# dusk-network/plonk

Hardware: NVIDIA H100
Metric: proofs/sec @ 2^16 gates (higher is better)
Workload: dtype u32 limbs (Fr 256-bit / Fp 384-bit Montgomery)

## Files before the change

### plonk_b200/csrc/msm.cu

```cuda
#include <algorithm>
#include <atomic>
#include <vector>

#include "common.cuh"
#include "fp_inv.cuh"
#include "g1.cuh"
#include "host_field.h"

struct pb200_srs {
  size_t n_points;
  int c;
  int W;
  uint4* table;
};

namespace pb {

static constexpr int kGroup = 8;
static constexpr unsigned kHeavyMin = 32, kHeavyFactor = 4;
static constexpr unsigned kHeavyChunk = 256, kHeavyChunkWide = 1024;

PB_D G1Affine ld_affine(const uint4* p, size_t i) {
  const uint4* q = p + 6 * i;
  uint4 a0 = __ldg(q), a1 = __ldg(q + 1), a2 = __ldg(q + 2), b0 = __ldg(q + 3), b1 = __ldg(q + 4), b2 = __ldg(q + 5);
  G1Affine r;
  r.x.v[0] = a0.x; r.x.v[1] = a0.y; r.x.v[2] = a0.z; r.x.v[3] = a0.w;
  r.x.v[4] = a1.x; r.x.v[5] = a1.y; r.x.v[6] = a1.z; r.x.v[7] = a1.w;
  r.x.v[8] = a2.x; r.x.v[9] = a2.y; r.x.v[10] = a2.z; r.x.v[11] = a2.w;
  r.y.v[0] = b0.x; r.y.v[1] = b0.y; r.y.v[2] = b0.z; r.y.v[3] = b0.w;
  r.y.v[4] = b1.x; r.y.v[5] = b1.y; r.y.v[6] = b1.z; r.y.v[7] = b1.w;
  r.y.v[8] = b2.x; r.y.v[9] = b2.y; r.y.v[10] = b2.z; r.y.v[11] = b2.w;
  return r;
}
PB_D void st_fp(uint4* q, const Fp& f) {
  q[0] = make_uint4(f.v[0], f.v[1], f.v[2], f.v[3]);
  q[1] = make_uint4(f.v[4], f.v[5], f.v[6], f.v[7]);
  q[2] = make_uint4(f.v[8], f.v[9], f.v[10], f.v[11]);
}
PB_D Fp ld_fp(const uint4* q) {
  uint4 a = q[0], b = q[1], c = q[2];
  Fp f;
  f.v[0] = a.x; f.v[1] = a.y; f.v[2] = a.z; f.v[3] = a.w;
  f.v[4] = b.x; f.v[5] = b.y; f.v[6] = b.z; f.v[7] = b.w;
  f.v[8] = c.x; f.v[9] = c.y; f.v[10] = c.z; f.v[11] = c.w;
  return f;
}
PB_D void st_affine(uint4* p, size_t i, const G1Affine& a) {
  st_fp(p + 6 * i, a.x);
  st_fp(p + 6 * i + 3, a.y);
}
PB_D void st_xyzz(uint4* p, size_t i, const G1Xyzz& a) {
  st_fp(p + 12 * i, a.x);
// ... 162 lines not shown
  s = s.from_mont();
  const unsigned mask = (1u << c) - 1u, half = 1u << (c - 1);
  unsigned carry = 0;
  for (int w = 0; w < W; w++) {
    const int bit = w * c;
    const int word = bit >> 5, off = bit & 31;
    unsigned val = 0;
    if (word < 8) {
      val = s.v[word] >> off;
      if (off && word + 1 < 8) val |= s.v[word + 1] << (32 - off);
      val &= mask;
    }
    unsigned d = val + carry;
    unsigned sign = 0;
    if (d > half) {
      d = (1u << c) - d;
      sign = 1;
      carry = 1;
    } else {
      carry = 0;
    }
    const size_t slot = ((size_t)b * W + w) * n + i;
    if (d == 0) {
      ebkt[slot] = 0xffffffffu;
    } else {
      const unsigned bucket = d - 1;
      ebkt[slot] = (bucket << 1) | sign;
      epos[slot] = atomicAdd(&counts[(size_t)b * nb + bucket], 1u);
    }
  }
}

__global__ void __launch_bounds__(1024) k_msm_scan(const unsigned* counts, unsigned* offsets, unsigned* order, unsigned* n_heavy,
                                                   unsigned* heavy_pre, unsigned* max_len, unsigned nb, int size_shift,
                                                   unsigned heavy_chunk) {
  __shared__ unsigned sums[1024];
  __shared__ unsigned bins[1024];
  __shared__ unsigned s_nh, s_total, s_thr_units, s_max;
  const unsigned b = blockIdx.x, tid = threadIdx.x;
  const unsigned* cnt = counts + (size_t)b * nb;
  unsigned* off = offsets + (size_t)b * (nb + 1);
  unsigned* ord = order + (size_t)b * nb;
  const unsigned chunk = (nb + 1023) / 1024;
  const unsigned lo = tid * chunk, hi = min(nb, lo + chunk);
  unsigned s = 0, mx = 0;
  for (unsigned k = lo; k < hi; k++) {
    s += cnt[k];
    mx = max(mx, cnt[k]);
  }
  sums[tid] = s;
  bins[tid] = 0;
  if (tid == 0) s_max = 0;
  __syncthreads();
  if (mx) atomicMax(&s_max, mx);
  for (unsigned d = 1; d < 1024; d <<= 1) {
    unsigned v = (tid >= d) ? sums[tid - d] : 0;
    __syncthreads();
    sums[tid] += v;
    __syncthreads();
  }
  unsigned run = sums[tid] - s;
  for (unsigned k = lo; k < hi; k++) {
    off[k] = run;
    run += cnt[k];
  }
  if (tid == 1023) {
    off[nb] = sums[1023];
    s_total = sums[1023];
    max_len[b] = s_max;
  }
  for (unsigned k = tid; k < nb; k += 1024) atomicAdd(&bins[1023u - min(cnt[k] >> size_shift, 1023u)], 1u);
  __syncthreads();
  const unsigned mine = bins[tid];
  sums[tid] = mine;
  __syncthreads();
  for (unsigned d = 1; d < 1024; d <<= 1) {
    unsigned v = (tid >= d) ? sums[tid - d] : 0;
    __syncthreads();
    sums[tid] += v;
    __syncthreads();
  }
  bins[tid] = sums[tid] - mine;
  if (tid == 0) {
    const unsigned avg = s_total / nb;
    const unsigned thr = max(kHeavyMin, kHeavyFactor * avg);
    s_thr_units = min(1021u, (thr + (1u << size_shift) - 1u) >> size_shift);
  }
  __syncthreads();
  if (tid == 1022u - s_thr_units) {
    n_heavy[b] = sums[tid];
    s_nh = sums[tid];
  }
  __syncthreads();
  for (unsigned k = tid; k < nb; k += 1024) {
    const unsigned pos = atomicAdd(&bins[1023u - min(cnt[k] >> size_shift, 1023u)], 1u);
    ord[pos] = k;
  }
  __syncthreads();
  const unsigned nh = s_nh;
  unsigned* hp = heavy_pre + (size_t)b * (nb + 1);
  const unsigned per = (nh + 1023u) / 1024u;
  const unsigned h_lo = min(nh, tid * per), h_hi = min(nh, h_lo + per);
  unsigned c = 0;
  for (unsigned h = h_lo; h < h_hi; h++) c += (cnt[ord[h]] + heavy_chunk - 1) / heavy_chunk;
  sums[tid] = c;
  __syncthreads();
  for (unsigned d = 1; d < 1024; d <<= 1) {
    unsigned v = (tid >= d) ? sums[tid - d] : 0;
    __syncthreads();
    sums[tid] += v;
    __syncthreads();
  }
  unsigned run2 = sums[tid] - c;
  for (unsigned h = h_lo; h < h_hi; h++) {
    hp[h] = run2;
    run2 += (cnt[ord[h]] + heavy_chunk - 1) / heavy_chunk;
  }
  if (tid == 1023) hp[nh] = sums[1023];
}

__global__ void k_msm_scatter(const unsigned* ebkt, const unsigned* epos, const unsigned* offsets, size_t n,
                              int W, unsigned nb, size_t n_table, size_t first, unsigned* sorted) {
  size_t i = (size_t)blockIdx.x * blockDim.x + threadIdx.x;
  if (i >= n) return;
  const unsigned w = blockIdx.y, b = blockIdx.z;
  const size_t slot = ((size_t)b * W + w) * n + i;
  const unsigned e = ebkt[slot];
  if (e == 0xffffffffu) return;
  const unsigned bucket = e >> 1, sign = e & 1u;
  const unsigned dst = offsets[(size_t)b * (nb + 1) + bucket] + epos[slot];
  sorted[(size_t)b * n * W + dst] = (unsigned)(((size_t)w * n_table + first + i) << 1) | sign;
}

PB_D G1Xyzz shfl_down_xyzz(const G1Xyzz& p, int delta, int width) {
  G1Xyzz r;
#pragma unroll
  for (int i = 0; i < 12; i++) {
    r.x.v[i] = __shfl_down_sync(0xffffffffu, p.x.v[i], delta, width);
    r.y.v[i] = __shfl_down_sync(0xffffffffu, p.y.v[i], delta, width);
    r.zz.v[i] = __shfl_down_sync(0xffffffffu, p.zz.v[i], delta, width);
    r.zzz.v[i] = __shfl_down_sync(0xffffffffu, p.zzz.v[i], delta, width);
  }
  return r;
}

template <int THREADS, int MIN_CTAS>
__global__ void __launch_bounds__(THREADS, MIN_CTAS) k_msm_accumulate(const uint4* table, const unsigned* sorted,
                                                               const unsigned* offsets, const unsigned* order,
                                                               const unsigned* n_heavy, unsigned nb, int log_split, size_t cap,
                                                               uint4* sums) {
  const size_t t = (size_t)blockIdx.x * blockDim.x + threadIdx.x;
  const unsigned split = 1u << log_split;
  const unsigned b = blockIdx.y;
  const bool valid = t < ((size_t)nb << log_split) && (t >> log_split) >= n_heavy[b];
  const unsigned part = (unsigned)t & (split - 1);
  unsigned bucket = 0, lo = 0, hi = 0;
  if (valid) {
    bucket = order[(size_t)b * nb + (t >> log_split)];
    const unsigned* off = offsets + (size_t)b * (nb + 1);
    const unsigned start = off[bucket], end = off[bucket + 1];
    const unsigned chunk = (end - start + split - 1) >> log_split;
    lo = min(end, start + part * chunk);
    hi = min(end, lo + chunk);
  }
  const unsigned* src = sorted + (size_t)b * cap;
  G1Xyzz acc = G1Xyzz::identity();
  unsigned e_next = 0;
  G1Affine p_next;
  if (lo < hi) {
    e_next = __ldg(src + lo);
    p_next = ld_affine(table, e_next >> 1);
  }
  for (unsigned k = lo; k < hi; k++) {
    const unsigned e = e_next;
    G1Affine p = p_next;
    if (k + 1 < hi) {
      e_next = __ldg(src + k + 1);
      p_next = ld_affine(table, e_next >> 1);
    }
    if (p.is_inf()) continue;
    if (e & 1u) p.y = p.y.neg();
    xyzz_madd(acc, p.x, p.y);
  }
  for (int d = (int)split >> 1; d > 0; d >>= 1) {
    G1Xyzz o = shfl_down_xyzz(acc, d, (int)split);
    xyzz_add(acc, o);
  }
  if (valid && part == 0) st_xyzz(sums, (size_t)b * nb + bucket, acc);
}

PB_D G1Xyzz warp_sum(G1Xyzz v) {
// ... 591 lines not shown
  *g_out = g;
  return 0;
}
static int msm_plan(const pb200_srs* srs, uint32_t batch, MsmTail* tail, unsigned* n_groups_out, int* g_out) {
  return msm_plan_c(srs->c, batch, tail, n_groups_out, g_out);
}

static unsigned reduction_chunks(const DigitPlan& plan, unsigned n_groups, unsigned n_parts) {
  unsigned chunks = (n_parts + kListChunk - 1) / kListChunk;
  for (int j = 0; j < plan.ndig; j++) chunks = std::max(chunks, ((n_groups >> plan.bits[j]) + kListChunk - 1) / kListChunk);
  return std::max(chunks, 1u);
}

static int msm_enqueue(const pb200_srs* srs, size_t first, const uint64_t* d_scalars, size_t n, uint32_t batch, size_t stride,
                       cudaStream_t st, ScratchScope& scope, uint4** d_result, MsmTail* tail, cudaEvent_t* prof_ev,
                       const unsigned** d_totals) {
  if (first + n > srs->n_points) return fail(PB200_ERR_DEGREE_TOO_LARGE, "more scalars than commit-key points");
  const int c = srs->c, W = srs->W;
  const unsigned nb = 1u << (c - 1);
  const size_t cap = n * (size_t)W;
  if (((srs->n_points * (size_t)W) << 1) >= ((size_t)1 << 32)) return fail(PB200_ERR_INVALID_ARG, "commit key too large for 32-bit point references");
  unsigned n_groups = 0;
  int g = 0;
  PB_TRY(msm_plan(srs, batch, tail, &n_groups, &g));
  const DigitPlan& plan = tail->plan;
  uint4* result = nullptr;
  PB_ALLOC(scope, result, (size_t)batch * (plan.ndig + 1) * 192);
  *d_result = result;
  if (n == 0) {
    PB_CUDA(cudaMemsetAsync(result, 0, (size_t)batch * (plan.ndig + 1) * 192, st));
    return 0;
  }

  int log_split = 0;
  if (!t_msm_throughput_hint) {
    const size_t avg = cap / nb;
    while (log_split < 5 && ((size_t)nb * batch << log_split) < (1u << 17) && (avg >> (log_split + 1)) >= 8) log_split++;
  }
  if (const char* env = getenv("PB200_MSM_LOG_SPLIT")) log_split = atoi(env);

  unsigned *counts = nullptr, *offsets = nullptr, *order = nullptr, *ebkt = nullptr, *epos = nullptr, *sorted = nullptr;
  uint4 *sums = nullptr, *lists = nullptr, *S = nullptr, *P = nullptr;
  PB_ALLOC(scope, counts, (size_t)batch * nb * 4);
  PB_ALLOC(scope, offsets, (size_t)batch * (nb + 1) * 4);
  PB_ALLOC(scope, order, (size_t)batch * nb * 4);
  const bool affine = msm_affine_enabled();
  unsigned *n_heavy = nullptr, *heavy_pre = nullptr, *max_len = nullptr;
  PB_ALLOC(scope, max_len, (size_t)batch * 4);
  PB_ALLOC(scope, n_heavy, (size_t)batch * 4);
  PB_ALLOC(scope, heavy_pre, (size_t)batch * (nb + 1) * 4);
  PB_ALLOC(scope, ebkt, (size_t)batch * cap * 4);
  PB_ALLOC(scope, epos, (size_t)batch * cap * 4);
  PB_ALLOC(scope, sorted, (size_t)batch * cap * 4);
  PB_ALLOC(scope, sums, (size_t)batch * nb * 192);
  const unsigned col_run = std::min(kColRun, n_groups), n_parts = n_groups / col_run;
  const unsigned chunks = reduction_chunks(plan, n_groups, n_parts);
  PB_ALLOC(scope, lists, (size_t)batch * plan.nlists * chunks * 192);
  PB_ALLOC(scope, S, (size_t)batch * n_groups * 192);
  PB_ALLOC(scope, P, (size_t)batch * g * n_parts * 192);
  PB_CUDA(cudaMemsetAsync(counts, 0, (size_t)batch * nb * 4, st));

  PB_LAUNCH(k_msm_digits, dim3(div_up(n, 128), batch), 128, 0, st, (const uint4*)d_scalars, n, stride, c, W, nb,
            counts, ebkt, epos);
  int size_shift = 0;
  while (((cap / nb) >> size_shift) > 64) size_shift++;
  const unsigned heavy_chunk = (t_msm_throughput_hint || t_msm_wide_heavy_chunks) ? kHeavyChunkWide : kHeavyChunk;
  const size_t part_cap = cap / kHeavyChunk + std::min<size_t>(nb, cap / kHeavyMin) + 2;
  uint4* partials = nullptr;
  PB_ALLOC(scope, partials, (size_t)batch * part_cap * 192);
  PB_LAUNCH(k_msm_scan, batch, 1024, 0, st, counts, offsets, order, n_heavy, heavy_pre, max_len, nb, size_shift, heavy_chunk);
  PB_LAUNCH(k_msm_scatter, dim3(div_up(n, 256), W, batch), 256, 0, st, ebkt, epos, offsets, n, W, nb,
            srs->n_points, first, sorted);
  if (prof_ev) PB_CUDA(cudaEventRecord(prof_ev[0], st));
  if (affine) {
    const size_t capA = cap / 2 + nb + 2, capB = cap / 4 + nb + 2;
    int rounds = 0;
    while (((size_t)1 << rounds) < cap) rounds++;
    auto positions = [&](int r) { return r == 0 ? cap : (cap >> r) + nb + 1; };
    const size_t slots = aff_slots(cap, nb);
    uint4 *bufA = nullptr, *bufB = nullptr, *pre = nullptr, *factor = nullptr, *ctot = nullptr, *cpre = nullptr;
    uint4* desc = nullptr;
    unsigned* npairs = nullptr;
    const size_t threads_max = slots / (kAffK / 2);
    const unsigned ctas_max = (unsigned)(threads_max / kAffThreads);
    PB_ALLOC(scope, bufA, (size_t)batch * capA * 96);
    PB_ALLOC(scope, bufB, (size_t)batch * capB * 96);
    PB_ALLOC(scope, pre, (size_t)batch * slots * 48);
    PB_ALLOC(scope, desc, (size_t)batch * slots * 16);
    PB_ALLOC(scope, factor, (size_t)batch * threads_max * 48);
    PB_ALLOC(scope, npairs, (size_t)batch * threads_max * 4);
    PB_ALLOC(scope, ctot, (size_t)batch * ctas_max * 48);
    PB_ALLOC(scope, cpre, (size_t)batch * ctas_max * 48);
    PB_CUDA(cudaMemsetAsync(sums, 0, (size_t)batch * nb * 96, st));
    for (int r = 0; r < rounds; r++) {
      AffRound a;
      a.table = srs->table; a.sorted = sorted; a.offsets = offsets; a.max_len = max_len; a.prefix = pre; a.desc = desc; a.sums = sums;
      a.factor = factor; a.ctot = ctot; a.npairs = npairs; a.ctas_max = ctas_max;
      a.nb = nb; a.cap = cap; a.r = r;
      a.in = (r & 1) ? bufA : bufB;
      a.out = (r & 1) ? bufB : bufA;
      a.in_cap = (r & 1) ? capA : capB;
      a.out_cap = (r & 1) ? capB : capA;
      const unsigned ctas = div_up(div_up(positions(r), kAffK), kAffThreads);
      a.threads = ctas * kAffThreads;
      a.slots = slots;
      const size_t stage_bytes = (size_t)kAffThreads * 15 * 16;
      if (r == 0)
        PB_LAUNCH(k_msm_affine_fwd<true>, dim3(ctas, batch), kAffThreads, 0, st, a);
      else
        PB_LAUNCH(k_msm_affine_fwd<false>, dim3(ctas, batch), kAffThreads, 0, st, a);
      PB_LAUNCH(k_fp_batch_inverse, batch, 256, 0, st, ctot, cpre, ctas, (size_t)ctas_max, (const unsigned*)max_len, r);
      if (r == 0)
        PB_LAUNCH(k_msm_affine_back<true>, dim3(ctas, batch), kAffThreads, stage_bytes, st, a);
      else
        PB_LAUNCH(k_msm_affine_back<false>, dim3(ctas, batch), kAffThreads, stage_bytes, st, a);
    }
    if (prof_ev) PB_CUDA(cudaEventRecord(prof_ev[1], st));
    if (d_totals) *d_totals = offsets + nb;
    PB_LAUNCH(k_msm_rows_cols<true>, dim3(div_up(n_groups + g * n_parts, 64), batch), 64, 0, st, (const uint4*)sums, nb, (unsigned)g, col_run, S, P);
  } else {
  {
    static const int acc_block = [] {
      const char* e = getenv("PB200_ACC_BLOCK");
      return e ? atoi(e) : 128;
    }();
    if (acc_block == 64) {
      const dim3 grid(div_up((size_t)nb << log_split, 64), batch);
      PB_LAUNCH((k_msm_accumulate<64, 4>), grid, 64, 0, st, srs->table, sorted, offsets, order, n_heavy, nb, log_split, cap, sums);
    } else {
      const dim3 grid(div_up((size_t)nb << log_split, 128), batch);
      PB_LAUNCH((k_msm_accumulate<128, 2>), grid, 128, 0, st, srs->table, sorted, offsets, order, n_heavy, nb, log_split, cap, sums);
    }
  }
  if (d_totals) *d_totals = offsets + nb;
  PB_LAUNCH(k_msm_heavy_chunks, dim3(4 * num_sms(), batch), 128, 0, st, srs->table, sorted, offsets, order, n_heavy, heavy_pre, nb, heavy_chunk, cap,
            part_cap, partials);
  PB_LAUNCH(k_msm_heavy_combine, dim3(64, batch), 128, 0, st, (const uint4*)partials, order, n_heavy, heavy_pre, nb, part_cap, sums);
  if (prof_ev) PB_CUDA(cudaEventRecord(prof_ev[1], st));
    PB_LAUNCH(k_msm_rows_cols<false>, dim3(div_up(n_groups + g * n_parts, 64), batch), 64, 0, st, (const uint4*)sums, nb, (unsigned)g, col_run, S, P);
  }
  PB_LAUNCH(k_msm_lists, dim3(div_up(plan.nlists, 4), batch, chunks), 128, 0, st, (const uint4*)S, (const uint4*)P, n_groups, n_parts, plan,
            chunks, lists);
  if (chunks > kFinalChunks) {
    PB_LAUNCH(k_msm_fold, div_up((size_t)batch * plan.nlists, 4), 128, 0, st, (const uint4*)lists, batch * (unsigned)plan.nlists, chunks, S);
    PB_LAUNCH(k_msm_final, batch, 256, 0, st, (const uint4*)S, plan, 1u, result);
  } else {
    PB_LAUNCH(k_msm_final, batch, 256, 0, st, (const uint4*)lists, plan, chunks, result);
  }
  PB_CUDA(cudaGetLastError());
  return 0;
}

static void msm_finish(const uint32_t* host, const MsmTail& tail, int n_parts, uint64_t* out_affine_host) {
  const DigitPlan& plan = tail.plan;
  const uint32_t batch = tail.batch;
  const size_t wpe = tail.words_per_entry();
  std::vector<pbh::HXyzz> res(batch);
  for (uint32_t b = 0; b < batch; b++) {
    auto digit = [&](int d) {
      pbh::HXyzz s = pbh::HXyzz::identity(), t;
      for (int p = 0; p < n_parts; p++) {
        xyzz_dev_to_host(host + ((size_t)p * batch + b) * wpe + (size_t)d * 48, &t);
        pbh::hxyzz_add(s, t);
      }
// ... 141 lines not shown
  if (e == cudaSuccess && *nccl_rc == 0) e = stream_wait(st);
  if (*nccl_rc != 0) return fail(PB200_ERR_CUDA, "ncclAllGather");
  PB_CUDA(e);
  scope.release();
  if (local_rc != 0) {
    g_last_error = local_msg;
    return local_rc;
  }
  std::vector<uint32_t> parts((size_t)n_ranks * payload / 4);
  for (int r = 0; r < n_ranks; r++) {
    const uint32_t* h = (const uint32_t*)(host + rec * (size_t)r);
    if (h[0] != 0) {
      char msg[48];
      snprintf(msg, sizeof msg, "rank %d", r);
      return fail(PB200_ERR_CUDA, "the partial MSM of another rank failed", msg);
    }
    if (h[1] != (uint32_t)tail.c || h[2] != (uint32_t)tail.plan.ndig || h[3] != batch)
      return fail(PB200_ERR_INVALID_ARG, "ranks disagree on the MSM window or batch (key slices must use one window width)");
    memcpy(parts.data() + (size_t)r * payload / 4, h + 4, payload);
  }
  msm_finish(parts.data(), tail, n_ranks, out_affine_host);
  return 0;
}

size_t msm_workspace_bytes(const pb200_srs* srs, size_t n, uint32_t batch) {
  const size_t nb = (size_t)1 << (srs->c - 1), cap = n * (size_t)srs->W;
  MsmTail tail;
  unsigned n_groups = 0;
  int g = 0;
  if (msm_plan(srs, batch, &tail, &n_groups, &g) != 0) return 0;
  const unsigned n_parts = n_groups / std::min(kColRun, n_groups);
  size_t b = 0;
  b += 4 * ((size_t)batch * (nb + 1) * 4 + 256);
  {
    int size_shift = 0;
    while (((cap / nb) >> size_shift) > 64) size_shift++;
    b += (size_t)batch * (cap / kHeavyChunk + std::min<size_t>(nb, cap / kHeavyMin) + 2) * 192 + 256;
  }
  b += (size_t)batch * 4 + 256;
  b += 3 * ((size_t)batch * cap * 4 + 256);
  b += (size_t)batch * nb * 192 + 256;
  b += (size_t)batch * n_groups * 192 + 256;
  b += (size_t)batch * g * n_parts * 192 + 256;
  b += (size_t)batch * tail.plan.nlists * reduction_chunks(tail.plan, n_groups, n_parts) * 192 + 256;
  b += (size_t)batch * 9 * 192 + 256;
  if (msm_affine_enabled()) {
    b += (size_t)batch * ((cap / 2 + nb + 2) + (cap / 4 + nb + 2)) * 96 + 512;
    b += (size_t)batch * aff_slots(cap, nb) * (48 + 16) + 512;
    b += (size_t)batch * (aff_slots(cap, nb) / (kAffK / 2)) * (48 + 4 + 1) + 2048;
  }
  return b + 4096;
}

int srs_upload(const uint8_t* raw, size_t n_points, pb200_srs** out, int window_bits) {
  if (n_points == 0) return fail(PB200_ERR_INVALID_ARG, "empty commit key");
  cudaStream_t st = thread_stream();
  pb200_srs* s = new pb200_srs();
  s->n_points = n_points;
  s->c = window_bits ? window_bits : pick_window(n_points);
  s->W = (256 + s->c - 1) / s->c;
  s->table = nullptr;
  cudaError_t e = cudaMalloc((void**)&s->table, (size_t)s->W * n_points * 96);
  if (e != cudaSuccess) {
    delete s;
    return fail(PB200_ERR_CUDA, "cudaMalloc(commit key table)", cudaGetErrorString(e));
  }
  e = cudaMemcpyAsync(s->table, raw, n_points * 96, cudaMemcpyHostToDevice, st);
  if (e == cudaSuccess) {
    PB_LAUNCH(k_msm_precompute, div_up(n_points, 64), 64, 0, st, s->table, n_points, s->c, s->W);
    e = cudaStreamSynchronize(st);
  }
  if (e != cudaSuccess) {
// ... 213 lines not shown
```

### plonk_b200/csrc/ntt.cu

```cuda
#include <cuda.h>

#include <mutex>
#include <vector>

#include "common.cuh"

namespace pb {

static constexpr int kMaxLogTile = 11;
static constexpr int kNttThreads = 256;

PB_D Fr ld_fr(const uint4* p, size_t i) {
  uint4 a = __ldg(p + 2 * i), b = __ldg(p + 2 * i + 1);
  Fr r;
  r.v[0] = a.x; r.v[1] = a.y; r.v[2] = a.z; r.v[3] = a.w;
  r.v[4] = b.x; r.v[5] = b.y; r.v[6] = b.z; r.v[7] = b.w;
  return r;
}
PB_D Fr ld_fr_nc(const uint4* p, size_t i) {
  uint4 a = p[2 * i], b = p[2 * i + 1];
  Fr r;
  r.v[0] = a.x; r.v[1] = a.y; r.v[2] = a.z; r.v[3] = a.w;
  r.v[4] = b.x; r.v[5] = b.y; r.v[6] = b.z; r.v[7] = b.w;
  return r;
// ... 201 lines not shown
  const size_t half_m = a.last ? 0 : ((size_t)1 << (a.r + a.log_lo - 1));
  for (int idx = tid; idx < (tile >> 1); idx += kNttThreads) {
    const int m = idx >> a.log_t, t = idx & (T - 1);
    const Fr x = tile_ld<TMA>(smem, tile, ((2 * m) << a.log_t) + t), y = tile_ld<TMA>(smem, tile, ((2 * m + 1) << a.log_t) + t);
    const int k0 = (int)(__brev((unsigned)(2 * m)) >> (32 - a.r));
    Fr v[2] = {x + y, x - y};
#pragma unroll
    for (int u = 0; u < 2; u++) {
      const int k = k0 + u * half_r;
      if (!a.last) {
        const size_t e = (size_t)k * (lo0 + t);
        Fr tw;
        if (e < half_m) {
          tw = ld_fr(a.w_m, e);
        } else {
          tw = ld_fr(a.w_m, e - half_m).neg();
        }
        st_fr(out, base + ((size_t)k << a.log_lo) + t, v[u] * tw);
      } else {
        const size_t o = (k0b + t) + (mid << a.log_r0) + ((size_t)k << a.log_h);
        Fr r = v[u];
        if (a.post) r = r * ld_fr(a.post, o);
        if (a.has_scalar) r = r * a.scalar;
        st_fr(out, o, r);
      }
    }
  }
}

struct PowArgs {
  Fr p2[32];
  Fr scale;
};
__global__ void k_powers(uint4* out, size_t n, PowArgs pa) {
  size_t i = (size_t)blockIdx.x * blockDim.x + threadIdx.x;
  if (i >= n) return;
  Fr acc = pa.scale;
  size_t e = i;
#pragma unroll 1
  for (int b = 0; b < 32 && e; b++, e >>= 1)
    if (e & 1) acc = acc * pa.p2[b];
  st_fr(out, i, acc);
}

static Fr fr_from_canonical(const uint32_t (&l)[8]) {
  Fr x;
  for (int i = 0; i < 8; i++) x.v[i] = l[i];
  return x.to_mont();
}
static const uint32_t kRootOfUnity[8] = {0x439f0d2bu, 0x3829971fu, 0x8c2280b9u, 0xb6368350u,
                                         0x22c813b4u, 0xd09b6819u, 0xdfe81f20u, 0x16a2a19eu};
static const uint32_t kGenerator[8] = {7, 0, 0, 0, 0, 0, 0, 0};

Fr ntt_group_gen(int log_n, bool inverse) {
  Fr g = fr_from_canonical(kRootOfUnity);
  for (int i = log_n; i < 32; i++) g = g.sqr();
  return inverse ? g.inv() : g;
}
static Fr ntt_size_inv_compute(int log_n) {
  uint32_t l[8] = {0, 0, 0, 0, 0, 0, 0, 0};
  l[log_n / 32] = 1u << (log_n % 32);
  Fr x;
  for (int i = 0; i < 8; i++) x.v[i] = l[i];
  return x.to_mont().inv();
}
Fr ntt_size_inv(int log_n) {
  static Fr cache[32];
  static std::once_flag once;
  std::call_once(once, [] {
    for (int i = 0; i < 32; i++) cache[i] = ntt_size_inv_compute(i);
  });
  return cache[log_n];
}
Fr ntt_coset_gen(bool inverse) {
  Fr g = fr_from_canonical(kGenerator);
  return inverse ? g.inv() : g;
}

struct TableCache {
  std::mutex mu;
  uint4* w[2][33] = {};
  uint4* coset_fwd = nullptr;
  size_t coset_fwd_len = 0;
  uint4* coset_inv[33] = {};
};
static TableCache g_tables;

int fill_powers(uint4* out, size_t n, const Fr& base, const Fr& scale, cudaStream_t st) {
  PowArgs pa;
  Fr p = base;
  for (int b = 0; b < 32; b++) {
    pa.p2[b] = p;
    p = p.sqr();
  }
  pa.scale = scale;
  PB_LAUNCH(k_powers, div_up(n, 256), 256, 0, st, out, n, pa);
  PB_CUDA(cudaGetLastError());
  return 0;
}

static int build_powers(uint4** out, size_t n, const Fr& base, const Fr& scale, cudaStream_t st) {
  PB_CUDA(cudaMalloc((void**)out, n * 32));
  PowArgs pa;
  Fr p = base;
  for (int b = 0; b < 32; b++) {
    pa.p2[b] = p;
    p = p.sqr();
  }
  pa.scale = scale;
  PB_LAUNCH(k_powers, div_up(n, 256), 256, 0, st, *out, n, pa);
  PB_CUDA(cudaGetLastError());
  return 0;
}

int get_twiddles(int logm, bool inverse, cudaStream_t st, const uint4** out) {
  std::lock_guard<std::mutex> lk(g_tables.mu);
  uint4*& slot = g_tables.w[inverse ? 1 : 0][logm];
  if (!slot) {
    size_t n = logm >= 1 ? ((size_t)1 << (logm - 1)) : 1;
    PB_TRY(build_powers(&slot, n, ntt_group_gen(logm, inverse), Fr::one(), st));
    PB_CUDA(cudaStreamSynchronize(st));
  }
  *out = slot;
  return 0;
}
static int get_coset_fwd(size_t n, cudaStream_t st, const uint4** out) {
  std::lock_guard<std::mutex> lk(g_tables.mu);
  if (g_tables.coset_fwd_len < n) {
    uint4* fresh = nullptr;
    PB_TRY(build_powers(&fresh, n, ntt_coset_gen(false), Fr::one(), st));
    PB_CUDA(cudaStreamSynchronize(st));
    g_tables.coset_fwd = fresh;
    g_tables.coset_fwd_len = n;
  }
  *out = g_tables.coset_fwd;
  return 0;
}
static int get_coset_inv(int log_n, cudaStream_t st, const uint4** out) {
  std::lock_guard<std::mutex> lk(g_tables.mu);
  uint4*& slot = g_tables.coset_inv[log_n];
  if (!slot) {
    PB_TRY(build_powers(&slot, (size_t)1 << log_n, ntt_coset_gen(true), ntt_size_inv(log_n), st));
    PB_CUDA(cudaStreamSynchronize(st));
// ... 145 lines not shown
```

### plonk_b200/csrc/prover.cu

```cuda
#include <algorithm>
#include <mutex>
#include <vector>

#include "common.cuh"
#include "host_field.h"
#include "plonk_algebra.cuh"
#include "transcript.h"

struct pb200_srs;

namespace pb {

int ntt_run(const uint64_t* d_in, size_t in_len, uint64_t* d_out, uint32_t log_n, int inverse, int coset,
            uint32_t batch, size_t in_stride, size_t out_stride, cudaStream_t st, Arena* ar);
int msm_run(const pb200_srs* srs, size_t first, const uint64_t* d_scalars, size_t n, uint32_t batch,
            size_t stride, uint64_t* out_affine_host, cudaStream_t st, Arena* ar);
size_t msm_workspace_bytes(const pb200_srs* srs, size_t n, uint32_t batch);
int srs_upload(const uint8_t* raw, size_t n_points, pb200_srs** out);
void srs_free(pb200_srs* s);
size_t srs_len(const pb200_srs* s);
const uint4* srs_points(const pb200_srs* s);
int srs_from_device(const uint4* d_points, size_t n_points, pb200_srs** out, int window_bits);
int msm_window_for(size_t n_points);
extern thread_local int t_msm_throughput_hint;
// ... 86 lines not shown
  stg_fr(p, i, x.to_mont());
}

__global__ void k_zero(uint4* p, size_t n_elems) {
  size_t i = (size_t)blockIdx.x * blockDim.x + threadIdx.x;
  if (i < n_elems) stg_fr(p, i, Fr::zero());
}

__global__ void k_sigma_lagrange(const unsigned long long* sig, size_t n, const uint4* w_half, uint4* out) {
  size_t i = (size_t)blockIdx.x * blockDim.x + threadIdx.x;
  if (i >= 4 * n) return;
  const unsigned long long e = sig[i];
  const unsigned col = (unsigned)(e >> 40);
  const size_t idx = (size_t)(e & 0xffffffffffull);
  Fr root = (idx < n / 2 || n == 1) ? ldg_fr(w_half, idx) : ldg_fr(w_half, idx - n / 2).neg();
  const uint32_t ks[4] = {1, 7, 13, 17};
  stg_fr(out, i, root * fr_small(ks[col]));
}

__global__ void k_perm_terms(const uint4* wv, const uint4* sigma, const uint4* w_half, size_t n, Fr beta, Fr gamma,
                             uint4* num, uint4* den) {
  size_t i = (size_t)blockIdx.x * blockDim.x + threadIdx.x;
  if (i >= n) return;
  Fr root = (i < n / 2 || n == 1) ? ldg_fr(w_half, i) : ldg_fr(w_half, i - n / 2).neg();
  Fr br = beta * root;
  Fr a = ldg_fr(wv, i), b = ldg_fr(wv, n + i), c = ldg_fr(wv, 2 * n + i), d = ldg_fr(wv, 3 * n + i);
  Fr nu = (a + br + gamma) * (b + br * fr_small(7) + gamma) * (c + br * fr_small(13) + gamma) * (d + br * fr_small(17) + gamma);
  Fr de = (a + beta * ldg_fr(sigma, i) + gamma) * (b + beta * ldg_fr(sigma, n + i) + gamma) *
          (c + beta * ldg_fr(sigma, 2 * n + i) + gamma) * (d + beta * ldg_fr(sigma, 3 * n + i) + gamma);
  stg_fr(num, i, nu);
  stg_fr(den, i, de);
}

__global__ void k_batch_div(const uint4* a, const uint4* b, size_t n, uint4* out) {
  const size_t t = (size_t)blockIdx.x * blockDim.x + threadIdx.x;
  const size_t base = t * 8;
  if (base >= n) return;
  Fr x[8], p[8];
  Fr acc = Fr::one();
#pragma unroll
  for (int k = 0; k < 8; k++) {
    x[k] = (base + k < n) ? ld_fr_plain(b, base + k) : Fr::one();
    if (!x[k].is_zero()) acc = acc * x[k];
    p[k] = acc;
  }
  Fr inv = acc.inv();
#pragma unroll
  for (int k = 7; k >= 0; k--) {
    if (base + k >= n) continue;
    Fr r;
    if (x[k].is_zero()) {
      r = Fr::zero();
    } else {
      r = (k > 0) ? inv * p[k - 1] : inv;
      inv = inv * x[k];
    }
    if (a) r = r * ld_fr_plain(a, base + k);
    stg_fr(out, base + k, r);
  }
}

template <bool MUL>
PB_D Fr scan_op(const Fr& a, const Fr& b) {
  return MUL ? a * b : a + b;
}
template <bool MUL>
PB_D Fr scan_id() {
  return MUL ? Fr::one() : Fr::zero();
}

template <bool MUL, bool REV>
__global__ void __launch_bounds__(256) k_scan_local(const uint4* in, size_t n, uint4* out, uint4* totals) {
  __shared__ uint4 sh[2][256][2];
  const int tid = threadIdx.x;
  const size_t base = ((size_t)blockIdx.x * 256 + tid) * 8;
  Fr p[8];
  Fr acc = scan_id<MUL>();
#pragma unroll
  for (int k = 0; k < 8; k++) {
// ... 449 lines not shown
    }
    PB_TRY(ntt_run((const uint64_t*)cols, n, (uint64_t*)P->d_polys, log_n, 1, 0, N_POLY, n, n, st, nullptr));
    {
      std::vector<uint64_t> aff((size_t)N_POLY * 12);
      PB_TRY(msm_run(P->srs, 0, (const uint64_t*)P->d_polys, n, N_POLY, n, aff.data(), st, nullptr));
      for (int k = 0; k < N_POLY; k++) compress_affine(aff.data() + 12 * k, P->comm[k]);
      const int widget_sel[4] = {Q_RANGE, Q_LOGIC, Q_FIXED, Q_VAR};
      for (int w = 0; w < 4; w++) P->has_widget[w] = (P->comm[widget_sel[w]][0] & 0x40) ? 0 : 1;
    }
  }
  PB_TRY(ntt_run((const uint64_t*)P->d_polys, n, (uint64_t*)P->d_key8, log_n + 3, 0, 1, N_POLY, n, n8, st, nullptr));
  {
    HFr lin[2] = {HFr::zero(), HFr::one()};
    PoolBlock lin_block(st);
    PB_CUDA(lin_block.alloc(64));
    uint4* d_lin = (uint4*)lin_block.p;
    PB_CUDA(cudaMemcpyAsync(d_lin, lin, 64, cudaMemcpyHostToDevice, st));
    PB_TRY(ntt_run((const uint64_t*)d_lin, 2, (uint64_t*)P->d_linear8, log_n + 3, 0, 1, 1, 2, n8, st, nullptr));
    PB_CUDA(cudaStreamSynchronize(st));
  }
  {
    const HFr g = to_host(ntt_coset_gen(false)), w8n = to_host(ntt_group_gen(log_n + 3, false));
    HFr point = g.pow_u64(n), step = w8n.pow_u64(n);
    const HFr psi = to_host(ntt_size_inv(log_n + 3)) * HFr::from_u64(8);
    Period8 c;
    for (int i = 0; i < 8; i++) {
      const HFr vh = point - HFr::one();
      P->vh_inv[i] = vh.inv();
      c.c[i] = to_dev(vh * psi);
      point = point * step;
    }
    PB_CUDA(cudaMemcpyAsync(P->d_l1_8, P->d_linear8, n8 * 32, cudaMemcpyDeviceToDevice, st));
    PB_LAUNCH(k_sub_one, div_up(n8, 256), 256, 0, st, P->d_l1_8, n8);
    PB_LAUNCH(k_batch_div, div_up(div_up(n8, 8), 128), 128, 0, st, (const uint4*)nullptr, (const uint4*)P->d_l1_8, n8, P->d_l1_8);
    PB_LAUNCH(k_scale_period8, div_up(n8, 256), 256, 0, st, P->d_l1_8, n8, c);
  }
  {
    P->edwards_d = to_dev(pbh::edwards_d());
    const HFr g = to_host(ntt_coset_gen(false)), w8n = to_host(ntt_group_gen(log_n + 3, false));
    const HFr h = g * w8n, w8r = w8n.pow_u64(n), wn = to_host(ntt_group_gen(log_n, false)), g4n = g.pow_u64(4 * n);
    HFr xs[16];
    xs[0] = h;
    for (int k = 1; k < 8; k++) xs[k] = xs[k - 1] * w8r;
    for (int k = 0; k < 8; k++) xs[8 + k] = xs[k] * wn;
    for (int k = 0; k < 16; k++) P->q4.xs[k] = to_dev(xs[k]);
    P->q4.fix.c = to_dev((g4n.dbl().neg()).inv());
    P->q4.fix.g4n = to_dev(g4n);
    const HFr h_inv = h.inv(), w8i = w8r.inv();
    HFr hj = HFr::from_u64(8).inv(), wp = HFr::one();
    for (int j = 0; j < 8; j++) {
      P->q4.fix.hinv8[j] = to_dev(hj);
      P->q4.fix.w8inv_pow[j] = to_dev(wp);
      hj = hj * h_inv;
      wp = wp * w8i;
    }
  }
  PB_TRY(ntt_run((const uint64_t*)(P->d_polys + 2 * (size_t)S1 * n), n, (uint64_t*)P->d_sigma, log_n, 0, 0, 4, n, n, st, nullptr));
  PB_CUDA(cudaGetLastError());
  PB_CUDA(cudaStreamSynchronize(st));
  {
    const size_t stride = n + 8;
    const size_t elems = 8 * n + 16 * stride + 64 * n + 64 + 16 * (size_t)div_up(stride, 2048) + 4 * (size_t)div_up(stride, 2048);
    const size_t ntt_tmp = 6 * n8 * 32;
    size_t msm_ws = msm_workspace_bytes(P->srs, std::min(stride, srs_len(P->srs)), 4);
    if (P->srs_lag) msm_ws = std::max(msm_ws, msm_workspace_bytes(P->srs_lag, n + 4, 4));
    P->ws_bytes = elems * 32 + std::max(ntt_tmp, msm_ws) + (size_t)64 * 256 + (1 << 20);
  }
// ... 180 lines not shown
  }
  PB_CUDA(cudaMemsetAsync(zp, 0, 6 * stride * 32, st));
  PB_TRY(ntt_run((const uint64_t*)wv, n, (uint64_t*)wp, log_n, 1, 0, n_pi ? 5 : 4, n, stride, st, ar));
  {
    BlindArgs ba;
    ba.nb = 2;
    ba.npoly = 4;
    for (int p = 0; p < 4; p++)
      for (int i = 0; i < 2; i++) ba.b[p][i] = to_dev(BL[2 * p + i]);
    PB_LAUNCH(k_blind, 1, 32, 0, st, wp, stride, n, ba);
  }
  if (P->srs_lag) {
    uint4* sc = w8;
    PB_CUDA(cudaMemcpy2DAsync(sc, stride * 32, wv, n * 32, n * 32, 4, cudaMemcpyDeviceToDevice, st));
    BlindArgs ba;
    ba.nb = 2;
    ba.npoly = 4;
    for (int p = 0; p < 4; p++)
      for (int i = 0; i < 2; i++) ba.b[p][i] = to_dev(BL[2 * p + i]);
    PB_LAUNCH(k_lagrange_tail, 1, 32, 0, st, sc, stride, n, ba);
    t_msm_throughput_hint = 0;
    t_msm_wide_heavy_chunks = (hint_at > 0 && (g_force_throughput.load(std::memory_order_relaxed) || P->active.load(std::memory_order_relaxed) >= hint_at)) ? 1 : 0;
    PB_TRY(msm_run(P->srs_lag, 0, (const uint64_t*)sc, n + 4, 4, stride, aff, st, ar));
    t_msm_wide_heavy_chunks = 0;
  } else {
    t_msm_throughput_hint = (hint_at > 0 && (g_force_throughput.load(std::memory_order_relaxed) || P->active.load(std::memory_order_relaxed) >= hint_at)) ? 1 : 0;
    PB_TRY(msm_run(P->srs, 0, (const uint64_t*)wp, n + 2, 4, stride, aff, st, ar));
  }
  for (int k = 0; k < 4; k++) compress_affine(aff + 12 * k, c48[C_A + k]);

  pbh::challenge_beta_gamma(tr, c48[0], ch);
  const HFr beta = ch.beta, gamma = ch.gamma;
  PB_LAUNCH(k_perm_terms, div_up(n, 128), 128, 0, st, (const uint4*)wv, (const uint4*)P->d_sigma, w_half, n, to_dev(beta), to_dev(gamma), num, den);
  PB_LAUNCH(k_batch_div, div_up(div_up(n, 8), 128), 128, 0, st, (const uint4*)num, (const uint4*)den, n, num);
  PB_TRY((fr_scan<true, false>(num, n, den, st, ar)));
  PB_TRY(ntt_run((const uint64_t*)den, n, (uint64_t*)zp, log_n, 1, 0, 1, n, stride, st, ar));
  {
    BlindArgs ba;
    ba.nb = 3;
    ba.npoly = 1;
    for (int i = 0; i < 3; i++) ba.b[0][i] = to_dev(BL[8 + i]);
    PB_LAUNCH(k_blind, 1, 32, 0, st, zp, stride, n, ba);
  }
  t_msm_throughput_hint = (hint_at > 0 && (g_force_throughput.load(std::memory_order_relaxed) || P->active.load(std::memory_order_relaxed) >= hint_at)) ? 1 : 0;
  PB_TRY(msm_run(P->srs, 0, (const uint64_t*)zp, n + 3, 1, stride, aff, st, ar));
  compress_affine(aff, c48[C_Z]);

  pbh::challenge_alpha(tr, c48[0], ch);
  const HFr alpha = ch.alpha;
  static const bool quot4n_env = [] {
    const char* e = getenv("PB200_QUOT4N");
    return !e || atoi(e) != 0;
  }();
  const bool quot4n = quot4n_env && n >= 16;
  const size_t n4 = 4 * n;
  size_t t_len = n8;
  QuotArgs q;
  {
    q.w8 = w8; q.key8 = P->d_key8; q.linear8 = P->d_linear8; q.l1_8 = P->d_l1_8; q.out = quot; q.n8 = n8;
    q.alpha = to_dev(alpha); q.beta = to_dev(beta); q.gamma = to_dev(gamma); q.alpha_sq = to_dev(alpha.sqr());
    auto powers = [](const HFr& c) {
      const SepPowers<HFr> h = sep_powers(c);
      SepPowers<Fr> s;
      s.ch = to_dev(h.ch); s.k = to_dev(h.k); s.k2 = to_dev(h.k2); s.k3 = to_dev(h.k3); s.k4 = to_dev(h.k4);
      return s;
    };
    q.ch_range = powers(ch.range); q.ch_logic = powers(ch.logic); q.ch_fixed = powers(ch.fixed); q.ch_var = powers(ch.var);
// ... 229 lines not shown
```

Before: 177.4.

## Adaptive per-bucket MSM split, block-level batch inversion, strided power generation

MSM accumulation now chooses a per-bucket split factor from each bucket's size class, computed in the scan kernel into a SplitPlan, instead of one global log_split. This is meant to balance lanes across uneven bucket sizes. k_batch_div now shares a single field inversion across a 256-thread block using warp shuffles and a shared prefix/suffix product, replacing one inversion per thread. k_powers computes 8 consecutive powers per thread by repeated multiplication, cutting the exponentiation work. Together these add more multiplications and synchronisation in exchange for fewer inversions and better MSM load balance.

```diff
diff --git a/plonk_b200/csrc/msm.cu b/plonk_b200/csrc/msm.cu
--- a/plonk_b200/csrc/msm.cu
+++ b/plonk_b200/csrc/msm.cu
@@ -6,6 +6,7 @@
 #include "fp_inv.cuh"
 #include "g1.cuh"
 #include "host_field.h"
+#include "msm_split.cuh"
 
 struct pb200_srs {
   size_t n_points;
@@ -17,7 +18,6 @@
 namespace pb {
 
 static constexpr int kGroup = 8;
-static constexpr unsigned kHeavyMin = 32, kHeavyFactor = 4;
 static constexpr unsigned kHeavyChunk = 256, kHeavyChunkWide = 1024;
 
 PB_D G1Affine ld_affine(const uint4* p, size_t i) {
@@ -246,11 +246,12 @@
 }
 
 __global__ void __launch_bounds__(1024) k_msm_scan(const unsigned* counts, unsigned* offsets, unsigned* order, unsigned* n_heavy,
-                                                   unsigned* heavy_pre, unsigned* max_len, unsigned nb, int size_shift,
-                                                   unsigned heavy_chunk) {
+                                                   unsigned* heavy_pre, unsigned* max_len, SplitPlan* plans, unsigned nb, int heavy_shift,
+                                                   int max_log, unsigned heavy_chunk) {
   __shared__ unsigned sums[1024];
   __shared__ unsigned bins[1024];
-  __shared__ unsigned s_nh, s_total, s_thr_units, s_max;
+  __shared__ unsigned s_nh, s_thr_units, s_max;
+  __shared__ unsigned s_split[kSplitRanges];
   const unsigned b = blockIdx.x, tid = threadIdx.x;
   const unsigned* cnt = counts + (size_t)b * nb;
   unsigned* off = offsets + (size_t)b * (nb + 1);
@@ -265,6 +266,7 @@
   sums[tid] = s;
   bins[tid] = 0;
   if (tid == 0) s_max = 0;
+  if (tid < kSplitRanges) s_split[tid] = 0;
   __syncthreads();
   if (mx) atomicMax(&s_max, mx);
   for (unsigned d = 1; d < 1024; d <<= 1) {
@@ -273,17 +275,18 @@
     sums[tid] += v;
     __syncthreads();
   }
+  const unsigned total = sums[1023];
   unsigned run = sums[tid] - s;
   for (unsigned k = lo; k < hi; k++) {
     off[k] = run;
     run += cnt[k];
   }
   if (tid == 1023) {
-    off[nb] = sums[1023];
-    s_total = sums[1023];
+    off[nb] = total;
     max_len[b] = s_max;
   }
-  for (unsigned k = tid; k < nb; k += 1024) atomicAdd(&bins[1023u - min(cnt[k] >> size_shift, 1023u)], 1u);
+  const int shift = msm_size_shift(total, nb);
+  for (unsigned k = tid; k < nb; k += 1024) atomicAdd(&bins[msm_sort_bin(cnt[k], shift)], 1u);
   __syncthreads();
   const unsigned mine = bins[tid];
   sums[tid] = mine;
@@ -295,23 +298,21 @@
     __syncthreads();
   }
   bins[tid] = sums[tid] - mine;
-  if (tid == 0) {
-    const unsigned avg = s_total / nb;
-    const unsigned thr = max(kHeavyMin, kHeavyFactor * avg);
-    s_thr_units = min(1021u, (thr + (1u << size_shift) - 1u) >> size_shift);
-  }
+  if (tid == 0) s_thr_units = msm_heavy_units(total, nb, shift, heavy_shift);
   __syncthreads();
   if (tid == 1022u - s_thr_units) {
     n_heavy[b] = sums[tid];
     s_nh = sums[tid];
   }
+  if (tid > 1022u - s_thr_units && mine) atomicAdd(&s_split[msm_log_split(1023u - tid, shift, max_log)], mine);
   __syncthreads();
   for (unsigned k = tid; k < nb; k += 1024) {
-    const unsigned pos = atomicAdd(&bins[1023u - min(cnt[k] >> size_shift, 1023u)], 1u);
+    const unsigned pos = atomicAdd(&bins[msm_sort_bin(cnt[k], shift)], 1u);
     ord[pos] = k;
   }
   __syncthreads();
   const unsigned nh = s_nh;
+  if (tid == 0) plans[b] = split_plan(s_split, nh);
   unsigned* hp = heavy_pre + (size_t)b * (nb + 1);
   const unsigned per = (nh + 1023u) / 1024u;
   const unsigned h_lo = min(nh, tid * per), h_hi = min(nh, h_lo + per);
@@ -361,16 +362,18 @@
 template <int THREADS, int MIN_CTAS>
 __global__ void __launch_bounds__(THREADS, MIN_CTAS) k_msm_accumulate(const uint4* table, const unsigned* sorted,
                                                                const unsigned* offsets, const unsigned* order,
-                                                               const unsigned* n_heavy, unsigned nb, int log_split, size_t cap,
-                                                               uint4* sums) {
-  const size_t t = (size_t)blockIdx.x * blockDim.x + threadIdx.x;
+                                                               const SplitPlan* plans, unsigned nb, size_t cap, uint4* sums) {
+  const unsigned t = blockIdx.x * blockDim.x + threadIdx.x;
+  const unsigned b = blockIdx.y;
+  const SplitPlan plan = plans[b];
+  unsigned idx = 0, part = 0;
+  int log_split = 0;
+  if (!split_plan_lane(plan, t, &idx, &log_split, &part)) return;
   const unsigned split = 1u << log_split;
-  const unsigned b = blockIdx.y;
-  const bool valid = t < ((size_t)nb << log_split) && (t >> log_split) >= n_heavy[b];
-  const unsigned part = (unsigned)t & (split - 1);
+  const bool valid = idx != kPadLane;
   unsigned bucket = 0, lo = 0, hi = 0;
   if (valid) {
-    bucket = order[(size_t)b * nb + (t >> log_split)];
+    bucket = order[(size_t)b * nb + idx];
     const unsigned* off = offsets + (size_t)b * (nb + 1);
     const unsigned start = off[bucket], end = off[bucket + 1];
     const unsigned chunk = (end - start + split - 1) >> log_split;
@@ -1028,12 +1031,7 @@
     return 0;
   }
 
-  int log_split = 0;
-  if (!t_msm_throughput_hint) {
-    const size_t avg = cap / nb;
-    while (log_split < 5 && ((size_t)nb * batch << log_split) < (1u << 17) && (avg >> (log_split + 1)) >= 8) log_split++;
-  }
-  if (const char* env = getenv("PB200_MSM_LOG_SPLIT")) log_split = atoi(env);
+  const int max_log = msm_max_log_split(nb, batch, t_msm_throughput_hint != 0);
 
   unsigned *counts = nullptr, *offsets = nullptr, *order = nullptr, *ebkt = nullptr, *epos = nullptr, *sorted = nullptr;
   uint4 *sums = nullptr, *lists = nullptr, *S = nullptr, *P = nullptr;
@@ -1045,6 +1043,8 @@
   PB_ALLOC(scope, max_len, (size_t)batch * 4);
   PB_ALLOC(scope, n_heavy, (size_t)batch * 4);
   PB_ALLOC(scope, heavy_pre, (size_t)batch * (nb + 1) * 4);
+  SplitPlan* plans = nullptr;
+  PB_ALLOC(scope, plans, (size_t)batch * sizeof(SplitPlan));
   PB_ALLOC(scope, ebkt, (size_t)batch * cap * 4);
   PB_ALLOC(scope, epos, (size_t)batch * cap * 4);
   PB_ALLOC(scope, sorted, (size_t)batch * cap * 4);
@@ -1058,13 +1058,12 @@
 
   PB_LAUNCH(k_msm_digits, dim3(div_up(n, 128), batch), 128, 0, st, (const uint4*)d_scalars, n, stride, c, W, nb,
             counts, ebkt, epos);
-  int size_shift = 0;
-  while (((cap / nb) >> size_shift) > 64) size_shift++;
+  const int heavy_shift = msm_size_shift((unsigned)cap, nb);
   const unsigned heavy_chunk = (t_msm_throughput_hint || t_msm_wide_heavy_chunks) ? kHeavyChunkWide : kHeavyChunk;
   const size_t part_cap = cap / kHeavyChunk + std::min<size_t>(nb, cap / kHeavyMin) + 2;
   uint4* partials = nullptr;
   PB_ALLOC(scope, partials, (size_t)batch * part_cap * 192);
-  PB_LAUNCH(k_msm_scan, batch, 1024, 0, st, counts, offsets, order, n_heavy, heavy_pre, max_len, nb, size_shift, heavy_chunk);
+  PB_LAUNCH(k_msm_scan, batch, 1024, 0, st, counts, offsets, order, n_heavy, heavy_pre, max_len, plans, nb, heavy_shift, max_log, heavy_chunk);
   PB_LAUNCH(k_msm_scatter, dim3(div_up(n, 256), W, batch), 256, 0, st, ebkt, epos, offsets, n, W, nb,
             srs->n_points, first, sorted);
   if (prof_ev) PB_CUDA(cudaEventRecord(prof_ev[0], st));
@@ -1120,12 +1119,13 @@
       const char* e = getenv("PB200_ACC_BLOCK");
       return e ? atoi(e) : 128;
     }();
+    const size_t threads = split_plan_max_threads(nb, max_log);
     if (acc_block == 64) {
-      const dim3 grid(div_up((size_t)nb << log_split, 64), batch);
-      PB_LAUNCH((k_msm_accumulate<64, 4>), grid, 64, 0, st, srs->table, sorted, offsets, order, n_heavy, nb, log_split, cap, sums);
+      const dim3 grid(div_up(threads, 64), batch);
+      PB_LAUNCH((k_msm_accumulate<64, 4>), grid, 64, 0, st, srs->table, sorted, offsets, order, (const SplitPlan*)plans, nb, cap, sums);
     } else {
-      const dim3 grid(div_up((size_t)nb << log_split, 128), batch);
-      PB_LAUNCH((k_msm_accumulate<128, 2>), grid, 128, 0, st, srs->table, sorted, offsets, order, n_heavy, nb, log_split, cap, sums);
+      const dim3 grid(div_up(threads, 128), batch);
+      PB_LAUNCH((k_msm_accumulate<128, 2>), grid, 128, 0, st, srs->table, sorted, offsets, order, (const SplitPlan*)plans, nb, cap, sums);
     }
   }
   if (d_totals) *d_totals = offsets + nb;
@@ -1333,12 +1333,9 @@
   const unsigned n_parts = n_groups / std::min(kColRun, n_groups);
   size_t b = 0;
   b += 4 * ((size_t)batch * (nb + 1) * 4 + 256);
-  {
-    int size_shift = 0;
-    while (((cap / nb) >> size_shift) > 64) size_shift++;
-    b += (size_t)batch * (cap / kHeavyChunk + std::min<size_t>(nb, cap / kHeavyMin) + 2) * 192 + 256;
-  }
+  b += (size_t)batch * (cap / kHeavyChunk + std::min<size_t>(nb, cap / kHeavyMin) + 2) * 192 + 256;
   b += (size_t)batch * 4 + 256;
+  b += (size_t)batch * sizeof(SplitPlan) + 256;
   b += 3 * ((size_t)batch * cap * 4 + 256);
   b += (size_t)batch * nb * 192 + 256;
   b += (size_t)batch * n_groups * 192 + 256;
diff --git a/plonk_b200/csrc/msm_split.cuh b/plonk_b200/csrc/msm_split.cuh
--- /dev/null
+++ b/plonk_b200/csrc/msm_split.cuh
@@ -0,0 +1,85 @@
+#pragma once
+#include <stddef.h>
+#include <stdint.h>
+
+#include "bigint.cuh"
+
+namespace pb {
+
+static constexpr unsigned kHeavyMin = 32, kHeavyFactor = 4;
+static constexpr unsigned kSortBins = 1024;
+static constexpr int kMaxLogSplit = 5;
+static constexpr int kSplitRanges = kMaxLogSplit + 1;
+static constexpr unsigned kMinPerLane = 8;
+static constexpr size_t kSplitLanes = (size_t)1 << 17;
+
+PB_HD int msm_size_shift(unsigned total, unsigned nb) {
+  int shift = 0;
+  while (((total / nb) >> shift) > 64) shift++;
+  return shift;
+}
+
+PB_HD unsigned msm_sort_bin(unsigned size, int shift) {
+  const unsigned units = size >> shift;
+  return kSortBins - 1u - (units < kSortBins - 1u ? units : kSortBins - 1u);
+}
+
+PB_HD unsigned msm_heavy_units(unsigned total, unsigned nb, int shift, int heavy_shift) {
+  const unsigned avg = total / nb, thr = kHeavyFactor * avg > kHeavyMin ? kHeavyFactor * avg : kHeavyMin;
+  unsigned units = (thr + (1u << heavy_shift) - 1u) >> heavy_shift;
+  if (units > kSortBins - 3u) units = kSortBins - 3u;
+  units = ((units + 1u) << (heavy_shift - shift)) - 1u;
+  return units < kSortBins - 3u ? units : kSortBins - 3u;
+}
+
+PB_HD int msm_max_log_split(unsigned nb, unsigned batch, bool throughput) {
+  int k = 0;
+  if (!throughput)
+    while (k < kMaxLogSplit && (((size_t)nb * batch) << k) < kSplitLanes) k++;
+  return k;
+}
+
+PB_HD int msm_log_split(unsigned units, int shift, int max_log) {
+  const size_t size = (size_t)units << shift;
+  int k = 0;
+  while (k < max_log && (size >> (k + 1)) >= kMinPerLane) k++;
+  return k;
+}
+
+struct SplitPlan {
+  unsigned pos[kSplitRanges + 1];
+  unsigned thr[kSplitRanges + 1];
+};
+
+PB_HD SplitPlan split_plan(const unsigned* count, unsigned n_heavy) {
+  SplitPlan p;
+  unsigned pos = n_heavy, thr = 0;
+  for (int r = 0; r < kSplitRanges; r++) {
+    const int k = kMaxLogSplit - r;
+    p.pos[r] = pos;
+    p.thr[r] = thr;
+    pos += count[k];
+    thr += ((count[k] << k) + 31u) & ~31u;
+  }
+  p.pos[kSplitRanges] = pos;
+  p.thr[kSplitRanges] = thr;
+  return p;
+}
+
+PB_HD size_t split_plan_max_threads(unsigned nb, int max_log) { return ((size_t)nb << max_log) + 32u * (max_log + 1); }
+
+static constexpr unsigned kPadLane = 0xffffffffu;
+
+PB_HD bool split_plan_lane(const SplitPlan& p, unsigned t, unsigned* idx, int* log_split, unsigned* part) {
+  if (t >= p.thr[kSplitRanges]) return false;
+  int r = 0;
+  while (t >= p.thr[r + 1]) r++;
+  const int k = kMaxLogSplit - r;
+  const unsigned local = t - p.thr[r], i = p.pos[r] + (local >> k);
+  *idx = i < p.pos[r + 1] ? i : kPadLane;
+  *log_split = k;
+  *part = local & ((1u << k) - 1u);
+  return true;
+}
+
+}
diff --git a/plonk_b200/csrc/ntt.cu b/plonk_b200/csrc/ntt.cu
--- a/plonk_b200/csrc/ntt.cu
+++ b/plonk_b200/csrc/ntt.cu
@@ -257,15 +257,20 @@
   Fr p2[32];
   Fr scale;
 };
+static constexpr unsigned kPowRun = 8;
 __global__ void k_powers(uint4* out, size_t n, PowArgs pa) {
-  size_t i = (size_t)blockIdx.x * blockDim.x + threadIdx.x;
-  if (i >= n) return;
+  const size_t i0 = ((size_t)blockIdx.x * blockDim.x + threadIdx.x) * kPowRun;
+  if (i0 >= n) return;
   Fr acc = pa.scale;
-  size_t e = i;
+  size_t e = i0;
 #pragma unroll 1
   for (int b = 0; b < 32 && e; b++, e >>= 1)
     if (e & 1) acc = acc * pa.p2[b];
-  st_fr(out, i, acc);
+#pragma unroll 1
+  for (unsigned k = 0; k < kPowRun && i0 + k < n; k++) {
+    if (k) acc = acc * pa.p2[0];
+    st_fr(out, i0 + k, acc);
+  }
 }
 
 static Fr fr_from_canonical(const uint32_t (&l)[8]) {
@@ -319,7 +324,7 @@
     p = p.sqr();
   }
   pa.scale = scale;
-  PB_LAUNCH(k_powers, div_up(n, 256), 256, 0, st, out, n, pa);
+  PB_LAUNCH(k_powers, div_up(div_up(n, kPowRun), 256), 256, 0, st, out, n, pa);
   PB_CUDA(cudaGetLastError());
   return 0;
 }
@@ -333,7 +338,7 @@
     p = p.sqr();
   }
   pa.scale = scale;
-  PB_LAUNCH(k_powers, div_up(n, 256), 256, 0, st, *out, n, pa);
+  PB_LAUNCH(k_powers, div_up(div_up(n, kPowRun), 256), 256, 0, st, *out, n, pa);
   PB_CUDA(cudaGetLastError());
   return 0;
 }
diff --git a/plonk_b200/csrc/prover.cu b/plonk_b200/csrc/prover.cu
--- a/plonk_b200/csrc/prover.cu
+++ b/plonk_b200/csrc/prover.cu
@@ -142,10 +142,24 @@
   stg_fr(den, i, de);
 }
 
-__global__ void k_batch_div(const uint4* a, const uint4* b, size_t n, uint4* out) {
+PB_D Fr shfl_up_fr(const Fr& a, int d) {
+  Fr r;
+#pragma unroll
+  for (int i = 0; i < 8; i++) r.v[i] = __shfl_up_sync(0xffffffffu, a.v[i], d);
+  return r;
+}
+PB_D Fr shfl_down_fr(const Fr& a, int d) {
+  Fr r;
+#pragma unroll
+  for (int i = 0; i < 8; i++) r.v[i] = __shfl_down_sync(0xffffffffu, a.v[i], d);
+  return r;
+}
+
+static constexpr unsigned kBatchDivThreads = 256;
+__global__ void __launch_bounds__(kBatchDivThreads) k_batch_div(const uint4* a, const uint4* b, size_t n, uint4* out) {
+  __shared__ uint4 sh_tot[kBatchDivThreads / 32 * 2];
   const size_t t = (size_t)blockIdx.x * blockDim.x + threadIdx.x;
   const size_t base = t * 8;
-  if (base >= n) return;
   Fr x[8], p[8];
   Fr acc = Fr::one();
 #pragma unroll
@@ -154,7 +168,36 @@
     if (!x[k].is_zero()) acc = acc * x[k];
     p[k] = acc;
   }
-  Fr inv = acc.inv();
+  const int lane = threadIdx.x & 31, warp = threadIdx.x >> 5;
+  Fr incl = acc, sfx = acc;
+#pragma unroll 1
+  for (int d = 1; d < 32; d <<= 1) {
+    const Fr up = shfl_up_fr(incl, d), dn = shfl_down_fr(sfx, d);
+    if (lane >= d) incl = incl * up;
+    if (lane + d < 32) sfx = sfx * dn;
+  }
+  Fr before = shfl_up_fr(incl, 1), after = shfl_down_fr(sfx, 1);
+  if (lane == 0) before = Fr::one();
+  if (lane == 31) after = Fr::one();
+  if (lane == 31) stg_fr(sh_tot, warp, incl);
+  __syncthreads();
+  if (threadIdx.x == 0) {
+    Fr w[kBatchDivThreads / 32], pf[kBatchDivThreads / 32];
+    Fr all = Fr::one();
+    for (unsigned k = 0; k < kBatchDivThreads / 32; k++) {
+      w[k] = ld_fr_plain(sh_tot, k);
+      pf[k] = all;
+      all = all * w[k];
+    }
+    Fr winv = all.inv();
+    for (int k = kBatchDivThreads / 32 - 1; k >= 0; k--) {
+      stg_fr(sh_tot, k, winv * pf[k]);
+      winv = winv * w[k];
+    }
+  }
+  __syncthreads();
+  if (base >= n) return;
+  Fr inv = ld_fr_plain(sh_tot, warp) * (before * after);
 #pragma unroll
   for (int k = 7; k >= 0; k--) {
     if (base + k >= n) continue;
@@ -670,7 +713,7 @@
     }
     PB_CUDA(cudaMemcpyAsync(P->d_l1_8, P->d_linear8, n8 * 32, cudaMemcpyDeviceToDevice, st));
     PB_LAUNCH(k_sub_one, div_up(n8, 256), 256, 0, st, P->d_l1_8, n8);
-    PB_LAUNCH(k_batch_div, div_up(div_up(n8, 8), 128), 128, 0, st, (const uint4*)nullptr, (const uint4*)P->d_l1_8, n8, P->d_l1_8);
+    PB_LAUNCH(k_batch_div, div_up(div_up(n8, 8), kBatchDivThreads), kBatchDivThreads, 0, st, (const uint4*)nullptr, (const uint4*)P->d_l1_8, n8, P->d_l1_8);
     PB_LAUNCH(k_scale_period8, div_up(n8, 256), 256, 0, st, P->d_l1_8, n8, c);
   }
   {
@@ -917,7 +960,7 @@
   pbh::challenge_beta_gamma(tr, c48[0], ch);
   const HFr beta = ch.beta, gamma = ch.gamma;
   PB_LAUNCH(k_perm_terms, div_up(n, 128), 128, 0, st, (const uint4*)wv, (const uint4*)P->d_sigma, w_half, n, to_dev(beta), to_dev(gamma), num, den);
-  PB_LAUNCH(k_batch_div, div_up(div_up(n, 8), 128), 128, 0, st, (const uint4*)num, (const uint4*)den, n, num);
+  PB_LAUNCH(k_batch_div, div_up(div_up(n, 8), kBatchDivThreads), kBatchDivThreads, 0, st, (const uint4*)num, (const uint4*)den, n, num);
   PB_TRY((fr_scan<true, false>(num, n, den, st, ar)));
   PB_TRY(ntt_run((const uint64_t*)den, n, (uint64_t*)zp, log_n, 1, 0, 1, n, stride, st, ar));
   {
```

After: 180.7, median of 6. +1.9%, better.
